# wild-firefox/FreeRL

Hardware: AMD Instinct MI355X
Metric: learner_updates_per_sec (higher is better)
Workload: dtype f32; 1 GPU; TD3.learn() (BASELINE configs[1] algorithm; north_star synthetic shape): obs_dim 8, act_dim 2, batch 256, replay 1e6 rows filled, hidden 128, policy_freq 2, device-drawn indices/noise; learners_per_gpu=512, kernel_family=chained (one eight-wave workgroup per learner, two waves per SIMD), rows_per_workgroup=256, lds_bytes=160128, parallelism=seeds sharded over 1 GPU(s), no data-path collective, collective=metric all-reduce: none (single process)

## Files before the change

### freerl_amd/csrc/frl_api.hip

```cpp
#include <hip/hip_runtime.h>

#include <chrono>
#include <cmath>
#include <cstdarg>
#include <cstdio>
#include <cstdlib>
#include <cstring>
#include <string>
#include <vector>

#include "../../include/freerl_hip.h"
#include "frl_desc.h"

#include "kernels.h"
#ifdef FRL_UNITY
#include "kernels_replay.hip"
#include "kernels_update.hip"
#include "kernels_dqn.hip"
#include "kernels_critic.hip"
#include "kernels_actor.hip"
#include "kernels_act.hip"
#include "kernels_ppo.hip"
#include "kernels_ppo2.hip"
#include "kernels_critic2.hip"
// ... 21 lines not shown
    va_start(ap, fmt);
    vsnprintf(buf, sizeof buf, fmt, ap);
    va_end(ap);
    g_err = buf;
    return code;
}

#define HIP_TRY(expr)                                                                              \
    do {                                                                                           \
        hipError_t _e = (expr);                                                                    \
        if (_e != hipSuccess) return fail(FRL_ERR_HIP, "%s: %s (%s:%d)", #expr, hipGetErrorString(_e), __FILE__, __LINE__); \
    } while (0)

static inline int pad16(int x) { return (x + 15) / 16 * 16; }
static inline int pad32(int x) { return (x + 31) / 32 * 32; }

struct frl_engine {
    frl_config cfg;
    EngineDesc h;
    EngineDesc* d = nullptr;
    hipStream_t stream = nullptr;
    hipEvent_t ev0 = nullptr, ev1 = nullptr, ev_stage = nullptr;
    int lds_bytes = 0;
    std::vector<int> index, size;
    float* stage_rows = nullptr;
    long long* stage_slots = nullptr;
    float* d_stage_rows = nullptr;
    long long* d_stage_slots = nullptr;
    int stage_cap = 0, stage_n = 0;
    bool stage_inflight = false;
    std::vector<int> staged_per_learner;
    int* h_idx = nullptr;
    long long* h_idx64 = nullptr;
    long long* d_idx64 = nullptr;
    float* h_noise = nullptr;
    size_t idx_count = 0, noise_count = 0;
    unsigned long long rng_counter = 0;
    float* d_act_wk = nullptr;
    size_t act_wk_slot = 0;
    std::vector<unsigned long long> act_wk_version;
    unsigned long long param_version = 1;
    float* d_solo_slab = nullptr;
    float* d_solo_part = nullptr;
    unsigned* d_solo_bar = nullptr;
    int* d_solo_err = nullptr;
    int* d_solo_pre = nullptr;
    unsigned solo_pre_seq = 0;
    bool ma_pre_valid = false;
    unsigned long long ma_pre_counter = 0;
    int ma_pre_size = 0, ma_pre_batch = 0;
    int* h_solo_err = nullptr;
    int* d_solo_ticket = nullptr;
    unsigned solo_bar_base = 0;
    int solo_stride = 0;
    int solow_wgs = 0;
    unsigned* d_solow_bar2 = nullptr;
    int solow_row_wgs = 0;
    float* d_act_in = nullptr;
    float* d_act_eps = nullptr;
    float* d_act_out = nullptr;
    float* d_act_logp = nullptr;
    size_t act_in_cap = 0, act_out_cap = 0;
    float* d_ou = nullptr;
    unsigned char* d_ou_flags = nullptr;
    size_t ou_n = 0;
    float* d_ppo = nullptr;
    size_t ppo_cap = 0;
    int* d_perm = nullptr;
    size_t perm_cap = 0;
    bool has_nets = false;
    int noisy_per_set = 0;
    float* h_noisy = nullptr;
    bool per_on = false;
    double* d_per_sum = nullptr;
    double* d_per_max = nullptr;
    float per_alpha = 0.5f, per_eps = 0.01f;
    double per_beta = 0.4, per_beta_inc = 0.001;
    std::vector<int> bucket_cursor;
    std::vector<int> size_flushed;
    int* d_size = nullptr;
    int n_cus = 256;
    int lds_per_cu = 160 * 1024;
    int chain_waves = 8;
    int* stage_bucket = nullptr;
    int* d_stage_bucket = nullptr;
    float* d_per_prio = nullptr;
    double* d_uniforms = nullptr;
    bool profile = false;
    std::vector<hipEvent_t> prof_ev;
    std::vector<int> prof_kind;
    size_t prof_used = 0;
    double prof_ms[8] = {0, 0, 0, 0, 0, 0, 0, 0};
    long long prof_n[8] = {0, 0, 0, 0, 0, 0, 0, 0};
};

enum ProfKind { PK_DRAW = 0, PK_GRAD_CRITIC = 1, PK_ADAM_CRITIC = 2, PK_GRAD_ACTOR = 3, PK_ADAM_ACTOR = 4, PK_SOFT = 5, PK_PPO = 6 };

static void prof_begin(frl_engine* e, int kind) {
    if (!e->profile) return;
    if (e->prof_used + 2 > e->prof_ev.size()) {
        for (int i = 0; i < 2; ++i) { hipEvent_t ev; hipEventCreate(&ev); e->prof_ev.push_back(ev); }
    }
    hipEventRecord(e->prof_ev[e->prof_used], e->stream);
    e->prof_kind.push_back(kind);
}
static void prof_end(frl_engine* e) {
    if (!e->profile) return;
    hipEventRecord(e->prof_ev[e->prof_used + 1], e->stream);
    e->prof_used += 2;
}
static void prof_collect(frl_engine* e) {
    if (e->prof_used == 0) return;
    hipStreamSynchronize(e->stream);
    for (size_t i = 0; i < e->prof_used; i += 2) {
        float ms = 0.f;
        if (hipEventElapsedTime(&ms, e->prof_ev[i], e->prof_ev[i + 1]) == hipSuccess) {
            const int k = e->prof_kind[i / 2];
            e->prof_ms[k] += ms;
            e->prof_n[k]++;
        }
    }
    e->prof_used = 0;
    e->prof_kind.clear();
}

static int build_net(NetDesc& N, const std::vector<std::pair<int, int>>& layers_in , int heads,
                     int hidden_act, int out_act, int extra_n, int n_shadow = 0) {
    memset(&N, 0, sizeof N);
    std::vector<std::pair<int, int>> layers = layers_in;
    for (int i = 0; i < n_shadow; ++i) layers.push_back(layers_in.back());
    N.n_layers = (int)layers.size();
    N.heads = heads;
    N.hidden_act = hidden_act;
    N.out_act = out_act;
    int off = 0, np = 0;
    for (int i = 0; i < N.n_layers; ++i) {
        LayerDesc& L = N.L[i];
        L.n = layers[i].first;
        L.k = layers[i].second;
        L.n_pad = pad16(L.n);
        L.k_pad = pad16(L.k);
        L.w_off = off;
        off += L.n_pad * L.k_pad;
        L.b_off = off;
        off += L.n_pad;
        np += L.n * L.k + L.n;
    }
    N.extra_off = -1;
    N.extra_n = extra_n;
    if (extra_n > 0) {
        N.extra_off = off;
        off += pad16(extra_n);
        np += extra_n;
    }
    N.size = pad32(off);
    N.n_params = np;
    N.n_layers -= n_shadow;
    N.n_shadow = n_shadow;
    return 0;
}

static void build_record(RecordDesc& R, const frl_config& c) {
    memset(&R, 0, sizeof R);
    R.n_agents = c.n_agents;
    int off = 0;
    for (int j = 0; j < c.n_agents; ++j) { R.obs_off[j] = off; R.obs_dim[j] = c.obs_dim[j]; off += c.obs_dim[j]; }
// ... 1073 lines not shown
}

extern "C" int frl_noisy_resample(frl_engine* e, const float* eps_host) {
    ENG(e);
    if (!e->h.noisy) return fail(FRL_ERR_STATE, "engine has no NoisyLinear head");
    if (eps_host) { int rc = noisy_upload(e, eps_host, 0, 1); if (rc) return rc; }
    else hipLaunchKernelGGL(noisy_draw_kernel, dim3(e->h.P, 1), dim3(256), 0, e->stream, e->d, 0, 1, e->rng_counter++);
    hipLaunchKernelGGL(noisy_materialise_kernel, dim3(e->h.P), dim3(256), 0, e->stream, e->d, 0, 1, 0);
    HIP_TRY(hipGetLastError());
    return FRL_OK;
}

static void launch_adam(frl_engine* e, hipStream_t st, const AdamArgs& ad, int units, dim3 grid_adam) {
    const EngineDesc& h = e->h;
    int max_n4 = 0;
    for (int ag = 0; ag < h.n_agents; ++ag) {
        const int net = (h.algo == ALGO_DQN) ? 0 : (ad.which == 0 ? 2 * ag + 1 : 2 * ag);
        max_n4 = std::max(max_n4, h.net[net].size / 4);
    }
    const bool two_pass = getenv("FRL_ADAM_TWO_PASS") != nullptr;
    if (max_n4 <= kFusedThreads * kFusedVec && !h.noisy && !two_pass) {
        hipLaunchKernelGGL(adam_fused_kernel, dim3(units), dim3(kFusedThreads), 0, st, e->d, ad);
    } else if (max_n4 <= kFusedThreads * kFusedVecWide && !two_pass) {
        hipLaunchKernelGGL(adam_fused_wide_kernel, dim3(units), dim3(kFusedThreads), 0, st, e->d, ad);
    } else {
        hipLaunchKernelGGL(reduce_kernel, grid_adam, dim3(256), 0, st, e->d, ad);
        hipLaunchKernelGGL(adam_kernel, grid_adam, dim3(256), 0, st, e->d, ad);
    }
}

static bool chained_shape(const EngineDesc& h) {
    const NetDesc &NA0 = h.net[0], &NC0 = h.net[1];
    auto packed = [](const NetDesc& N) {
        for (int hd = 0; hd < N.heads; ++hd) {
            const LayerDesc* L = N.L + 3 * hd;
            const int b = hd * kHeadFloats;
            if (L[0].w_off != b + kL1w || L[0].b_off != b + kL1b || L[1].w_off != b + kL2w || L[1].b_off != b + kL2b ||
                L[2].w_off != b + kL3w || L[2].b_off != b + kL3b) return false;
        }
        return N.extra_n == 0 || (N.heads == 1 && N.extra_off == kHeadFloats);
    };
    if (NA0.n_layers != 3 || NC0.n_layers != 3 * NC0.heads || h.hidden != 128 || !packed(NA0) || !packed(NC0)) return false;
    if (h.rec.obs_off[0] % 4 != 0 || h.rec.act_off[0] != h.rec.obs_off[0] + h.rec.obs_dim[0] || h.rec.obs_off[0] + 16 > h.rec.stride) return false;
    return (h.algo == ALGO_DDPG || h.algo == ALGO_TD3 || h.algo == ALGO_SAC) && h.n_agents == 1 && h.hidden == 128 &&
           NA0.L[0].k_pad == 16 && NC0.L[0].k_pad == 16 && h.rec.act_dim[0] <= 4 && NA0.L[2].n_pad == 16 &&
           h.batch_max <= 256 && NA0.hidden_act == ACT_RELU && NC0.hidden_act == ACT_RELU &&
           NA0.n_layers == 3 && NC0.n_layers == 3 * NC0.heads;
}
static bool chained_path(const EngineDesc& h, int batch, int pc) {
    (void)pc;
    if (h.wide) return !h.obs_norm_on;
    if (h.solow) return !h.obs_norm_on;
    return h.net[0].frag && h.net[1].frag && batch <= 256 && !h.obs_norm_on;
}
static bool wide_shape(const EngineDesc& h) {
    const bool single = (h.algo == ALGO_DDPG || h.algo == ALGO_TD3 || h.algo == ALGO_SAC) && h.n_agents == 1;
    const bool multi = h.algo == ALGO_MADDPG && h.n_agents >= 1;
    const int H = h.hidden;
    if (!(single || multi) || (H != 128 && H != 256) || h.rec.act_total > kWideApitch) return false;
    if (h.batch_max > 2 * kWideSlice) return false;
    const int nt3 = h.net[0].L[2].n_pad;
    for (int j = 0; j < h.n_agents; ++j) {
        const NetDesc &NA0 = h.net[2 * j], &NC0 = h.net[2 * j + 1];
        if (NA0.n_layers != 3 || NA0.heads != 1 || NC0.n_layers != 3 * NC0.heads || NC0.heads != h.net[1].heads) return false;
        if (NA0.hidden_act != ACT_RELU || NC0.hidden_act != ACT_RELU) return false;
        if (NA0.L[0].k_pad > 16 * kWideMaxKB1 || NC0.L[0].k_pad > 16 * kWideMaxKB1) return false;
        if (NA0.L[2].n_pad != nt3 || nt3 > 32) return false;
        for (int hd = 0; hd < NC0.heads; ++hd)
            if (NC0.L[3 * hd].n_pad != H || NC0.L[3 * hd + 1].n_pad != H || NC0.L[3 * hd + 1].k_pad != H || NC0.L[3 * hd + 2].n_pad != 16) return false;
        if (NA0.L[0].n_pad != H || NA0.L[1].n_pad != H || NA0.L[1].k_pad != H) return false;
    }
    return true;
}

static bool dqn_fused_path(const EngineDesc& h, int batch, bool per_weights) {
    const NetDesc& N = h.net[0];
    (void)per_weights;
    const bool shape = h.algo == ALGO_DQN && !h.noisy && !h.c51_atoms && h.hidden == 128 && N.n_layers == 2 &&
                       N.L[0].k_pad == 16 && N.L[1].n_pad == 16 && batch <= kDqn2Batch && !h.obs_norm_on && N.hidden_act == ACT_RELU;
    const char* force = getenv("FRL_DQN_FUSED");
    return shape && (force ? atoi(force) != 0 : true);
}

static void launch_learn_stage(frl_engine* e, hipStream_t st, LearnArgs a, int stage, int p0, int pc, bool dev_rng, bool needs_noise,
                               const DqnStepArgs* step = nullptr, const SoloStepArgs* sstep = nullptr) {
    const EngineDesc& h = e->h;
    a.p0 = p0; a.p_count = pc;
    const int ns = ((a.batch + h.rc - 1) / h.rc + h.cps - 1) / h.cps;
    const int units = pc * h.n_agents;
    const dim3 grid_chunks(((units + 7) / 8) * 8 * ns), grid_units(units), blk(256), grid_adam(units * h.Gmax);
    const bool sac = h.algo == ALGO_SAC || h.algo == ALGO_SAC_DISCRETE, maddpg = h.algo == ALGO_MADDPG;
    AdamArgs ad;
    memset(&ad, 0, sizeof ad);
    ad.ns = ns; ad.batch = a.batch; ad.eps = a.adam_eps; ad.beta1 = a.beta1; ad.beta2 = a.beta2; ad.clip = a.clip_norm;
    ad.tau = a.tau; ad.alpha_lr = a.alpha_lr; ad.target_entropy = a.target_entropy; ad.p0 = p0; ad.G = h.Gmax;
    const bool v2 = chained_path(h, a.batch, pc);
    if (stage == 0 && dqn_fused_path(h, a.batch, a.use_isw != 0)) {
        a.dqn_split = dqn_split_for(h, a.batch, pc);
        prof_begin(e, PK_GRAD_CRITIC);
        DqnStepArgs sa;
        memset(&sa, 0, sizeof sa);
        if (step) sa = *step;
        hipLaunchKernelGGL(dqn_fused_kernel, dim3(pc * a.dqn_split), blk, (size_t)dqn2_lds_floats() * sizeof(float), st, e->d, a, sa);
        prof_end(e);
        return;
    }
    const int ma_pre_stride = 8 + h.batch_max;
    const bool ma_solow = v2 && h.solow && h.n_agents > 1 && stage == 0 && dev_rng && !needs_noise && pc == h.P;
    const bool ma_use_pre = ma_solow && e->ma_pre_valid && e->ma_pre_counter == a.rng_counter && e->ma_pre_size == a.size && e->ma_pre_batch == a.batch;
    if (stage == 0) {
        if (dev_rng && !ma_use_pre && !(v2 && (h.solo || (h.solow && h.n_agents == 1)))) {
            prof_begin(e, PK_DRAW);
            const char* scan = getenv("FRL_DRAW_SCAN");
            const bool table = a.batch > 256 && 4 * a.batch <= kDrawTableHost && !(scan && atoi(scan) != 0);
            const size_t draw_lds = ((size_t)2 * ((a.batch + 3) & ~3) + (table ? 2 * kDrawTableHost : 0)) * sizeof(int);
            hipLaunchKernelGGL(draw_kernel, grid_units, blk, draw_lds, st, e->d, a, (needs_noise ? 1 : 0) | (table ? 0 : 2));
            prof_end(e);
        }
        if (h.obs_norm_on && h.algo != ALGO_DQN)
            hipLaunchKernelGGL(obsnorm_kernel, dim3(pc), blk, 0, st, e->d, a.batch, 0, p0);
        if (h.noisy)
            hipLaunchKernelGGL(noisy_materialise_kernel, dim3(h.P), blk, 0, st, e->d, 0, 3, 0x2);
        if (v2 && h.wide) {
            prof_begin(e, PK_GRAD_CRITIC);
            const bool x = h.wide == 2;
            const size_t lb = (size_t)(x ? wide16_lds_floats_host() : wide_lds_floats()) * sizeof(float);
            const bool twin = h.net[1].heads == 2, a2 = h.net[0].L[2].n_pad > 16;
            auto k = x ? (twin ? (a2 ? ac_critic_x_h2a2_kernel : ac_critic_x_h2a1_kernel) : (a2 ? ac_critic_x_h1a2_kernel : ac_critic_x_h1a1_kernel))
                       : (twin ? (a2 ? ac_critic_wide_h2a2_kernel : ac_critic_wide_h2a1_kernel) : (a2 ? ac_critic_wide_h1a2_kernel : ac_critic_wide_h1a1_kernel));
            hipLaunchKernelGGL(k, dim3(units), blk, lb, st, e->d, a);
            prof_end(e);
            return;
        }
        if (v2 && h.solow) {
            prof_begin(e, PK_GRAD_CRITIC);
            SoloArgs sa{e->d_solo_slab, e->d_solo_part, e->d_solo_bar, e->d_solo_err, e->solo_bar_base, e->solo_stride, nullptr, nullptr, 0ull, h.solow, e->d_solow_bar2, e->solow_row_wgs, e->solow_wgs};
            e->solo_bar_base += kSoloWG;
            if (dev_rng && e->d_solo_pre && pc == h.P && h.n_agents == 1) {
                const char* pdf = getenv("FRL_SOLO_PREDRAW");
                sa.pre_read = e->d_solo_pre + (size_t)(e->solo_pre_seq & 1) * h.P * kSoloPre;
                if (e->solow_wgs > e->solow_row_wgs && !(pdf && atoi(pdf) == 0)) {
                    sa.pre_write = e->d_solo_pre + (size_t)((e->solo_pre_seq + 1) & 1) * h.P * kSoloPre;
                    sa.pre_counter = e->rng_counter;
                }
                ++e->solo_pre_seq;
            }
            const bool twin = h.net[1].heads == 2, a2 = h.net[0].L[2].n_pad > 16;
            auto k = h.n_agents > 1 ? (twin ? (a2 ? solow_critic_ma_h2a2_kernel : solow_critic_ma_h2a1_kernel) : (a2 ? solow_critic_ma_h1a2_kernel : solow_critic_ma_h1a1_kernel))
                                    : (twin ? (a2 ? solow_critic_h2a2_kernel : solow_critic_h2a1_kernel) : (a2 ? solow_critic_h1a2_kernel : solow_critic_h1a1_kernel));
            if (a.fuse_actor) k = twin ? (a2 ? solow_step_h2a2_kernel : solow_step_h2a1_kernel) : (a2 ? solow_step_h1a2_kernel : solow_step_h1a1_kernel);
            int extra = 0;
            if (h.n_agents > 1) {
                const char* pdf = getenv("FRL_SOLO_PREDRAW");
                if (ma_use_pre) sa.pre_read = e->d_solo_pre + (size_t)(e->solo_pre_seq & 1) * h.P * h.n_agents * ma_pre_stride;
                e->ma_pre_valid = false;
                if (ma_solow && units * (e->solow_wgs + 1) <= e->n_cus && !(pdf && atoi(pdf) == 0)) {
                    sa.pre_write = e->d_solo_pre + (size_t)((e->solo_pre_seq + 1) & 1) * h.P * h.n_agents * ma_pre_stride;
                    sa.pre_counter = e->rng_counter;
                    extra = units;
                    e->ma_pre_valid = true; e->ma_pre_counter = e->rng_counter; e->ma_pre_size = a.size; e->ma_pre_batch = a.batch;
                }
                ++e->solo_pre_seq;
            }
            hipLaunchKernelGGL(k, dim3(units * e->solow_wgs + extra), blk, (size_t)solow_lds_floats() * sizeof(float), st, e->d, a, sa);
            prof_end(e);
            return;
        }
        if (v2 && h.solo) {
            prof_begin(e, PK_GRAD_CRITIC);
            SoloArgs sa{e->d_solo_slab, e->d_solo_part, e->d_solo_bar, e->d_solo_err, e->solo_bar_base, e->solo_stride, nullptr, nullptr, 0ull};
            e->solo_bar_base += kSoloWG;
            SoloStepArgs ss;
            memset(&ss, 0, sizeof ss);
            if (sstep) ss = *sstep;
            const size_t lb = (size_t)std::max(solo_lds_floats(), critic2_lds_floats()) * sizeof(float);
            const char* pdf = getenv("FRL_SOLO_PREDRAW");
            const int W = h.solo;
            const bool predraw = dev_rng && !sstep && e->d_solo_pre && pc == h.P && pc * (W + 1) <= e->n_cus && !(pdf && atoi(pdf) == 0);
            int extra = 0;
            if (dev_rng && !sstep && e->d_solo_pre && pc == h.P) {
                sa.pre_read = e->d_solo_pre + (size_t)(e->solo_pre_seq & 1) * h.P * kSoloPre;
                if (predraw) {
                    sa.pre_write = e->d_solo_pre + (size_t)((e->solo_pre_seq + 1) & 1) * h.P * kSoloPre;
                    sa.pre_counter = e->rng_counter;
                    extra = pc;
                }
                ++e->solo_pre_seq;
            }
            const bool twin = h.net[1].heads == 2;
            auto k = W == 16 ? (twin ? solo_critic_twin_kernel : solo_critic_single_kernel) : (twin ? solo_critic_twin_w8_kernel : solo_critic_single_w8_kernel);
            hipLaunchKernelGGL(k, dim3(pc * W + extra), blk, lb, st, e->d, a, sa, ss);
            prof_end(e);
            return;
        }
        if (v2) {
            { const char* sg = getenv("FRL_STAGGER"); a.stagger = sg ? atoi(sg) : 0;
              const char* gg = getenv("FRL_STAGGER_GROUPS"); a.stagger_groups = gg ? atoi(gg) : 4; a.stagger_wgs = e->n_cus; }
            prof_begin(e, PK_GRAD_CRITIC);
            const bool w8 = e->chain_waves == 8, twin = h.net[1].heads == 2;
            const size_t lb = (size_t)(w8 ? critic8_lds_floats() : critic2_lds_floats()) * sizeof(float);
            const RecordDesc& R = h.rec;
            const bool nv = R.nobs_off[0] % 4 == 0 && R.nobs_off[0] + 16 <= R.stride && R.rew_off % 2 == 0 && R.done_off == R.rew_off + 1 && !getenv("FRL_CRITIC2_NOVEC");
            auto k = w8 ? (nv ? (twin ? ac_critic_v2_twin_nv_kernel : ac_critic_v2_single_nv_kernel) : (twin ? ac_critic_v2_twin_kernel : ac_critic_v2_single_kernel))
                        : (twin ? ac_critic_v2w4_twin_kernel : ac_critic_v2w4_single_kernel);
            hipLaunchKernelGGL(k, dim3(pc), dim3(w8 ? 512 : 256), lb, st, e->d, a);
            prof_end(e);
            return;
        }
        prof_begin(e, PK_GRAD_CRITIC);
        if (h.algo == ALGO_DQN && h.c51_atoms) hipLaunchKernelGGL(c51_grad_kernel, grid_chunks, blk, e->lds_bytes, st, e->d, a, ns);
        else if (h.algo == ALGO_DQN) hipLaunchKernelGGL(dqn_grad_kernel, grid_chunks, blk, e->lds_bytes, st, e->d, a, ns);
        else if (h.algo == ALGO_SAC_DISCRETE) hipLaunchKernelGGL(sacd_critic_kernel, grid_chunks, blk, e->lds_bytes, st, e->d, a, ns);
        else hipLaunchKernelGGL(ac_critic_kernel, grid_chunks, blk, e->lds_bytes, st, e->d, a, ns);
        prof_end(e);
        ad.which = 0; ad.lr = a.critic_lr; ad.wd = a.critic_wd;
        ad.soft = (h.algo == ALGO_DQN) ? 1 : ((!maddpg && a.do_actor) ? 1 : 0);
        prof_begin(e, PK_ADAM_CRITIC);
        launch_adam(e, st, ad, units, grid_adam);
        prof_end(e);
    } else if (stage == 1) {
        if (v2 && h.wide) {
            prof_begin(e, PK_GRAD_ACTOR);
            const bool x = h.wide == 2, a2 = h.net[0].L[2].n_pad > 16;
            auto k = x ? (a2 ? ac_actor_x_a2_kernel : ac_actor_x_a1_kernel) : (a2 ? ac_actor_wide_a2_kernel : ac_actor_wide_a1_kernel);
            hipLaunchKernelGGL(k, dim3(units), blk, (size_t)(x ? wide16_lds_floats_host() : wide_lds_floats()) * sizeof(float), st, e->d, a);
            prof_end(e);
            return;
        }
        if (v2 && h.solow) {
            prof_begin(e, PK_GRAD_ACTOR);
            SoloArgs sa{e->d_solo_slab, e->d_solo_part, e->d_solo_bar, e->d_solo_err, e->solo_bar_base, e->solo_stride, nullptr, nullptr, 0ull, h.solow, e->d_solow_bar2, e->solow_row_wgs, e->solow_wgs};
            e->solo_bar_base += kSoloWG;
            const bool a2 = h.net[0].L[2].n_pad > 16;
            hipLaunchKernelGGL(h.n_agents > 1 ? (a2 ? solow_actor_ma_a2_kernel : solow_actor_ma_a1_kernel) : (a2 ? solow_actor_a2_kernel : solow_actor_a1_kernel), dim3(units * e->solow_wgs), blk,
                               (size_t)solow_lds_floats() * sizeof(float), st, e->d, a, sa);
            prof_end(e);
            return;
        }
        if (v2 && h.solo) {
            prof_begin(e, PK_GRAD_ACTOR);
            SoloArgs sa{e->d_solo_slab, e->d_solo_part, e->d_solo_bar, e->d_solo_err, e->solo_bar_base, e->solo_stride, nullptr, nullptr, 0ull};
            e->solo_bar_base += kSoloWG;
            SoloStepArgs ss;
            memset(&ss, 0, sizeof ss);
            if (sstep) ss = *sstep;
            const int W = h.solo;
            hipLaunchKernelGGL(W == 16 ? solo_actor_kernel : solo_actor_w8_kernel, dim3(pc * W), blk,
                               (size_t)std::max(solo_lds_floats(), critic2_lds_floats()) * sizeof(float), st, e->d, a, sa, ss);
            prof_end(e);
            return;
        }
        if (v2) {
            prof_begin(e, PK_GRAD_ACTOR);
            const bool w8 = e->chain_waves == 8;
            hipLaunchKernelGGL(w8 ? ac_actor_v2_kernel : ac_actor_v2w4_kernel, dim3(pc), dim3(w8 ? 512 : 256),
                               (size_t)(w8 ? critic8_lds_floats() : critic2_lds_floats()) * sizeof(float), st, e->d, a);
            prof_end(e);
            return;
        }
        prof_begin(e, PK_GRAD_ACTOR);
        if (h.algo == ALGO_SAC_DISCRETE) hipLaunchKernelGGL(sacd_actor_kernel, grid_chunks, blk, e->lds_bytes, st, e->d, a, ns);
        else hipLaunchKernelGGL(ac_actor_kernel, grid_chunks, blk, e->lds_bytes, st, e->d, a, ns);
        prof_end(e);
        ad.which = 1; ad.lr = a.actor_lr; ad.wd = 0.f; ad.soft = maddpg ? 0 : 1; ad.sac_alpha = sac ? 1 : 0;
        prof_begin(e, PK_ADAM_ACTOR);
        launch_adam(e, st, ad, units, grid_adam);
        prof_end(e);
    } else {
        prof_begin(e, PK_SOFT);
        int biggest = 0;
        for (int i = 0; i < h.n_nets; ++i) biggest = std::max(biggest, h.net[i].size);
        const int per = std::max(1, std::min((biggest + 4095) / 4096, 4 * e->n_cus / std::max(1, pc * h.n_nets)));
        hipLaunchKernelGGL(soft_update_kernel, dim3(pc * h.n_nets, per), blk, 0, st, e->d, a.tau, p0);
        prof_end(e);
    }
}

static int learn_impl(frl_engine* e, const frl_learn_args* args, const DqnStepArgs* step, const SoloStepArgs* sstep = nullptr, int size_override = -1,
                      hipStream_t stream_override = nullptr) {
    ENG(e);
    if (!args) return fail(FRL_ERR_INVALID, "args is NULL");
    const EngineDesc& h = e->h;
    if (!(h.algo == ALGO_DQN || h.algo == ALGO_DDPG || h.algo == ALGO_TD3 || h.algo == ALGO_SAC || h.algo == ALGO_MADDPG ||
          h.algo == ALGO_SAC_DISCRETE))
        return fail(FRL_ERR_STATE, "frl_learn: engine algo %d has no off-policy learn (PPO: frl_ppo_learn)", h.algo);
    if (args->batch < 1 || args->batch > h.batch_max) return fail(FRL_ERR_INVALID, "batch %d outside [1,%d]", args->batch, h.batch_max);
    int min_size = h.capacity;
    for (int p = 0; p < h.P; ++p) min_size = std::min(min_size, e->size[p]);
    if (size_override >= 0) min_size = size_override;
    if (min_size < args->batch) return fail(FRL_ERR_STATE, "a ring holds %d rows < batch %d", min_size, args->batch);
    if (args->per && (h.algo != ALGO_DQN || !e->per_on)) return fail(FRL_ERR_STATE, "per = 1 needs a DQN engine with frl_per_enable");
    if (args->per && args->idx) return fail(FRL_ERR_INVALID, "per = 1 uses the rows of the last frl_per_sample; idx must be NULL");
    const bool dev_rng = (args->idx == nullptr) && !args->per;
    if (dev_rng && min_size < 2 * args->batch)
        return fail(FRL_ERR_STATE, "device index draw needs len(buffer) >= 2*batch (have %d); pass idx", min_size);
    const bool td3_like = (h.algo == ALGO_TD3 || h.algo == ALGO_MADDPG);
    const bool needs_noise = (h.algo == ALGO_SAC) || (td3_like && args->use_policy_noise);
    if (!dev_rng && needs_noise && !args->noise) return fail(FRL_ERR_INVALID, "idx given without noise: both or neither");
    int rc = flush_stage(e);
    if (rc) return rc;
    rc = upload_idx_noise(e, args->idx, needs_noise ? args->noise : nullptr, args->batch, h.n_agents);
    if (rc) return rc;
    LearnArgs a;
    memset(&a, 0, sizeof a);
    a.batch = args->batch;
    a.size = min_size;
    a.device_rng = dev_rng ? 1 : 0;
    a.do_actor = td3_like ? (args->do_actor ? 1 : 0) : 1;
    a.gamma = args->gamma; a.tau = args->tau;
    a.actor_lr = args->actor_lr; a.critic_lr = args->critic_lr; a.alpha_lr = args->alpha_lr;
    a.adam_eps = args->adam_eps > 0 ? args->adam_eps : 1e-8f;
    a.beta1 = 0.9f; a.beta2 = 0.999f;
    a.critic_wd = args->critic_weight_decay;
    a.clip_norm = args->clip_norm;
    a.policy_noise = args->policy_noise; a.noise_clip = args->noise_clip;
    a.max_action = args->max_action != 0.f ? args->max_action : 1.f;
    a.policy_noise_scale = args->policy_noise_scale;
    a.use_policy_noise = (td3_like && args->use_policy_noise) ? 1 : 0;
    a.target_entropy = args->target_entropy;
    a.double_dqn = (h.algo == ALGO_DQN && args->double_dqn) ? 1 : 0;
    a.use_isw = (h.algo == ALGO_DQN && args->per) ? (args->per == 2 ? 2 : 1) : 0;
    if (args->loss_kind != FRL_LOSS_MSE && args->loss_kind != FRL_LOSS_HUBER) return fail(FRL_ERR_INVALID, "unknown loss_kind %d", args->loss_kind);
    if (args->loss_kind == FRL_LOSS_HUBER) {
        if (!(args->huber_delta > 0.f)) return fail(FRL_ERR_INVALID, "Huber loss needs huber_delta > 0");
        if (h.c51_atoms) return fail(FRL_ERR_STATE, "the Categorical head's loss is a cross-entropy: no Huber variant");
        if (h.algo == ALGO_SAC_DISCRETE) return fail(FRL_ERR_INVALID, "discrete SAC's critic loss is F.mse_loss (SAC_add_discrete.py:313-314): no Huber variant");
        a.huber = 1; a.huber_delta = args->huber_delta;
    }
    a.rng_counter = e->rng_counter++;
    ++e->param_version;
    const bool actor_stage = (h.algo != ALGO_DQN && a.do_actor), soft_stage = (h.algo == ALGO_MADDPG && a.do_actor && !(h.solow && chained_path(h, a.batch, h.P)));
    if (h.noisy) {
        const int first = a.double_dqn ? 0 : 1;
        if (args->noisy_eps) { rc = noisy_upload(e, args->noisy_eps, first, 3 - first); if (rc) return rc; }
        else hipLaunchKernelGGL(noisy_draw_kernel, dim3(h.P, 3), dim3(256), 0, e->stream, e->d, 0, 3, e->rng_counter++);
// ... 323 lines not shown
```

### freerl_amd/csrc/frl_desc.h

```cpp
#pragma once
#include <stdint.h>

namespace frl {

constexpr int kMaxLayers = 6;
constexpr int kMaxAgents = 8;
constexpr int kMaxNets = 2 * kMaxAgents;

enum Act : int { ACT_NONE = 0, ACT_RELU = 1, ACT_TANH = 2 };
enum Algo : int { ALGO_DQN = 0, ALGO_DDPG = 1, ALGO_TD3 = 2, ALGO_SAC = 3, ALGO_MADDPG = 4, ALGO_PPO = 5, ALGO_SAC_DISCRETE = 6 };

struct LayerDesc {
    int n, k;
    int n_pad, k_pad;
    int w_off, b_off;
};

struct NetDesc {
    int n_layers;
    int size;
    int n_params;
    int hidden_act;
    int out_act;
    int extra_off;
// ... 55 lines not shown
};

struct EngineDesc {
    int algo, P, n_agents, hidden, rc;
    int capacity;
    int batch_max;
    int n_nets;
    int learner_stride;
    int net_off[kMaxNets];
    NetDesc net[kMaxNets];
    RecordDesc rec;
    float* theta;
    float* target;
    float* m;
    float* v;
    float* grad;
    float* slab;
    float* act_spill;
    float* part;
    int S;
    int cps;
    float* gsq;
    int Gmax;
    float* replay;
    int* idx;
    float* noise;
    int noise_sets;
    float* stats;
    int* steps;
    int* ticket;
    float* alpha;
    unsigned long long seed;
    int act_max;
    int lds_kin_pad, lds_out_pad, lds_batch_pad, lds_act_pad;
    int lds_hbufs;
    int n_discrete;
    float* isw;
    float* td_err;
    int noisy;
    int noisy_split;
    float* theta_eff;
    float* noisy_eps;
    int c51_atoms;
    float c51_vmin, c51_vmax;
    int dueling;
    int cat_logits;
    int beta_actor;
    float* obsnorm;
    int obs_norm_on;
    int obsnorm_w;
    int wide;
    int wide_bm;
    int wide_xp, wide_op;
    int wide_unit;
    float* wide_scr;
    int solow;
    int solo;
};

struct LearnArgs {
    int batch;
    int size;
    int device_rng;
    int do_actor;
    float gamma, tau;
    float actor_lr, critic_lr, alpha_lr;
    float adam_eps, beta1, beta2;
    float critic_wd;
    float clip_norm;
    float policy_noise, noise_clip, max_action, policy_noise_scale;
    int use_policy_noise;
    float target_entropy;
    unsigned long long rng_counter;
    int p0, p_count;
    int double_dqn;
    int use_isw;
    int dqn_split;
    int stagger;
    int stagger_groups;
    int stagger_wgs;
    int fuse_actor;
    int huber;
    float huber_delta;
};

}
```

### freerl_amd/csrc/kernels_actor2.hip

```cpp
#include <hip/hip_runtime.h>

#include "kernels.h"
#include "device/chain_net.hpp"
#include "device/update_common.hpp"
#include "device/ppo_timing.hpp"

namespace frl {

template <int NW, int TA>
__device__ __forceinline__ void ac_actor_v2_body(const EngineDesc& D, const LearnArgs& a, float* smem) {
    constexpr int kRC = 16 * NW, kRowsT = kRC * TA;
    constexpr int kNC = kChainBatch / kRC, kNCT = kChainBatch / kRowsT;
    static_assert(kNCT >= 1, "a chunk of passes A / B is at most the whole batch");
    const int p = a.p0 + blockIdx.x;
    const RecordDesc& R = D.rec;
    const NetDesc& NA = D.net[0];
    const NetDesc& NC = D.net[1];
    using Net = ChainNetT<NW>;
    Net C;
    C.init(smem);
    const ChainLds& S = C.S;
    const int tid = C.tid, l = C.l, w = C.w, i16 = C.i16, q = C.q;
    const int B = a.batch, O = R.obs_dim[0], A = R.act_dim[0];
    const size_t lbase = (size_t)p * D.learner_stride;
    g_f thA = as_global(D.theta + lbase + D.net_off[0]);
    g_f tgA = as_global(D.target + lbase + D.net_off[0]);
    g_f mA = as_global(D.m + lbase + D.net_off[0]);
    g_f vA = as_global(D.v + lbase + D.net_off[0]);
    g_cf thC = as_global(D.theta + lbase + D.net_off[1]);
    g_cf ring = as_global(D.replay + (size_t)p * D.capacity * R.stride);
    g_ci idx = as_global_i(D.idx + (size_t)p * D.batch_max);
    const float invB = 1.f / (float)B;
    const bool sac = (D.algo == ALGO_SAC);
    const float alpha = sac ? D.alpha[p * 4 + 3] : 0.f;
    const int am = D.act_max;
    g_cf noise1 = as_global(D.noise + ((size_t)p * D.noise_sets + 1) * D.batch_max * am);
    const int nq = sac ? NC.heads : 1;
    const float dqv = sac ? -0.5f * invB : -invB;
    const int nchunks = (B + kRC - 1) / kRC, nch2 = (B + kRowsT - 1) / kRowsT;
    lds_f dab = S.eb;

    int ridxT[kNC], ridx[kNC];
#pragma unroll
    for (int j4 = 0; j4 < kNC; ++j4) {
        const int rowT = (j4 / TA) * kRowsT + 16 * TA * w + (j4 % TA) * 16 + i16, row = j4 * kRC + 16 * w + i16;
        ridxT[j4] = rowT < B ? idx[rowT] : -1;
        ridx[j4] = row < B ? idx[row] : -1;
    }
    struct RowIn2 { f32x4 x[TA]; };
    auto load_obs2 = [&](int c2) {
        RowIn2 X;
#pragma unroll
        for (int t = 0; t < TA; ++t) {
            X.x[t] = f32x4{0.f, 0.f, 0.f, 0.f};
            int ri = ridxT[t];
#pragma unroll
            for (int cc = 1; cc < kNCT; ++cc) ri = c2 == cc ? ridxT[TA * cc + t] : ri;
            if (ri >= 0) {
                g_cf rec = ring + (size_t)ri * R.stride;
#pragma unroll
                for (int e = 0; e < 4; ++e)
                    if (4 * q + e < O) X.x[t][e] = rec[R.obs_off[0] + 4 * q + e];
            }
        }
        return X;
    };
    auto load_obs = [&](int c) {
        f32x4 x = {0.f, 0.f, 0.f, 0.f};
        const int ri = pick(ridx, c);
        if (ri >= 0) {
            g_cf rec = ring + (size_t)ri * R.stride;
#pragma unroll
            for (int e = 0; e < 4; ++e)
                if (4 * q + e < O) x[e] = rec[R.obs_off[0] + 4 * q + e];
        }
        return x;
    };

    float lpsum = 0.f;
    PPO_T0();
    RowIn2 nxt2 = load_obs2(0);
    typename Net::StageRegs pend = C.stage_fetch((g_cf)thA, 0, NA.extra_n);
    C.stage_commit(pend);
    PPO_T(0);
    for (int c2 = 0; c2 < nch2; ++c2) {
        const RowIn2 cur = nxt2;
        nxt2 = load_obs2(c2 + 1 < nch2 ? c2 + 1 : 0);
        if (c2 + 1 == nch2) pend = C.stage_fetch(thC, 0);
        f32x4 z[TA], h1[TA][kHT], h2[TA][kHT];
        C.template forward_vh<TA>(cur.x, h1, h2, z, A);
#pragma unroll
        for (int t = 0; t < TA; ++t) {
            const int row = c2 * kRowsT + 16 * TA * w + 16 * t + i16;
            if (q == 0 && row < kChainBatch) {
                f32x4 an = {0.f, 0.f, 0.f, 0.f};
#pragma unroll
                for (int r = 0; r < 4; ++r) {
                    if (r < A && row < B) {
                        if (sac) {
                            const float ls = fminf(fmaxf(S.ls[r], -20.f), 2.f), sd = expf(ls);
                            const float u = z[t][r] + sd * noise1[(size_t)row * am + r], du = u - z[t][r];
                            lpsum += -(du * du) / (2.f * sd * sd) - ls - kLogSqrt2Pi;
                            lpsum -= 2.f * (kLog2 - u - softplus_t(-2.f * u));
                            an[r] = tanhf(u);
                        } else {
                            an[r] = tanhf(z[t][r]);
                        }
                    }
                }
                st4(S.ab + row * 4, an);
            }
        }
    }
    float qsum = 0.f;
    f32x4 nxt;
    PPO_T(1);
    for (int hd = 0; hd < nq; ++hd) {
        C.stage_commit(pend);
        PPO_T(0);
        for (int c2 = 0; c2 < nch2; ++c2) {
            const RowIn2 cur = nxt2;
            if (c2 + 1 < nch2) nxt2 = load_obs2(c2 + 1);
            else if (hd + 1 < nq) nxt2 = load_obs2(0);
            else nxt = load_obs(0);
            f32x4 xb[TA], z[TA], h1[TA][kHT], h2[TA][kHT];
#pragma unroll
            for (int t = 0; t < TA; ++t) {
                const int row = c2 * kRowsT + 16 * TA * w + 16 * t + i16;
                xb[t] = cur.x[t];
#pragma unroll
                for (int e = 0; e < 4; ++e) {
                    const int f = 4 * q + e;
                    if (row < B && f >= O && f < O + A) xb[t][e] = S.ab[row * 4 + f - O];
                }
            }
            C.template forward_vh<TA>(xb, h1, h2, z, 1);
#pragma unroll
            for (int t = 0; t < TA; ++t) {
                const int row = c2 * kRowsT + 16 * TA * w + 16 * t + i16;
                const bool valid = row < B;
                f32x4 dz = {0.f, 0.f, 0.f, 0.f};
                if (q == 0 && valid) { qsum += z[t][0]; dz[0] = dqv; }
                f32x4 d2[kHT], d1[kHT];
                C.delta2_valu(dz, h2[t], d2, 1);
                C.delta1(d2, h1[t], d1);
                const f32x4 dx = C.delta0(d1);
#pragma unroll
                for (int r = 0; r < 4; ++r) {
                    const int f = 4 * q + r;
                    if (valid && f >= O && f < O + A) dab[row * 4 + f - O] = hd == 0 ? dx[r] : dab[row * 4 + f - O] + dx[r];
                }
            }
        }
        pend = hd + 1 < nq ? C.stage_fetch(thC, hd + 1) : C.stage_fetch((g_cf)thA, 0, NA.extra_n);
        PPO_T(2);
    }
    typename Net::Grad g;
    PPO_T(2);
    C.grad_zero(g);
    C.stage_commit(pend);
    PPO_T(0);
    f32x4 dqa[kNC], epsa[kNC], ava[NW == 8 ? kNC : 1];
#pragma unroll
    for (int c = 0; c < kNC; ++c) {
        const int row = c * kRC + 16 * w + i16;
        dqa[c] = (q == 0 && row < B) ? ld4((lds_cf)(dab + row * 4)) : f32x4{0.f, 0.f, 0.f, 0.f};
        if constexpr (NW == 8) ava[c] = (q == 0 && row < B) ? ld4((lds_cf)(S.ab + row * 4)) : f32x4{0.f, 0.f, 0.f, 0.f};
        epsa[c] = f32x4{0.f, 0.f, 0.f, 0.f};
        if (sac && q == 0 && row < B) {
#pragma unroll
            for (int r = 0; r < 4; ++r)
                if (r < A) epsa[c][r] = noise1[(size_t)row * am + r];
        }
    }
    float gls[4] = {0.f, 0.f, 0.f, 0.f};
    for (int c = 0; c < nchunks; ++c) {
        const int row = c * kRC + 16 * w + i16;
        f32x4 xb[1] = {nxt}, z[1], h1[1][kHT], h2[1][kHT];
        nxt = load_obs(c + 1 < nchunks ? c + 1 : 0);
        PPO_T(5);
        C.template forward_vh<1>(xb, h1, h2, z, A);
        PPO_T(3);
        const f32x4 dq = pick(dqa, c);
        f32x4 dz = {0.f, 0.f, 0.f, 0.f};
        if (q == 0 && row < B) {
            if (sac) {
                const f32x4 ep = pick(epsa, c);
                f32x4 av4;
                if constexpr (NW == 8) av4 = pick(ava, c); else av4 = ld4((lds_cf)(S.ab + row * 4));
#pragma unroll
                for (int r = 0; r < 4; ++r) {
                    if (r < A) {
                        const float av = av4[r];
                        const float d = dq[r] * (1.f - av * av) + (alpha * invB) * (2.f * av);
                        const float ls = fminf(fmaxf(S.ls[r], -20.f), 2.f);
                        dz[r] = d;
                        gls[r] += d * expf(ls) * ep[r] - alpha * invB;
                    }
                }
            } else {
#pragma unroll
                for (int r = 0; r < 4; ++r)
                    if (r < A) { const float av = tanhf(z[0][r]); dz[r] = dq[r] * (1.f - av * av); }
            }
        }
        C.backward(g, xb[0], h1[0], h2[0], dz, A);
        PPO_T(4);
    }
    C.grad_finish(g);
    float ss = wave_sum(C.grad_sumsq(g));
    const float qs = wave_sum(qsum), lps = wave_sum(lpsum);
#pragma unroll
    for (int r = 0; r < 4; ++r) gls[r] = wave_sum(gls[r]);
    lds_barrier();
    if (l == 0) {
        S.red[w] = ss; S.red[8 + w] = qs; S.red[16 + w] = lps;
#pragma unroll
        for (int r = 0; r < 4; ++r) S.red[24 + 8 * r + w] = gls[r];
    }
    int* steps = D.steps + (size_t)p * (kMaxNets + 1);
    if (tid == 0) S.red[56] = __int_as_float(steps[0]);
    lds_barrier();
    auto red_sum = [&](int base) {
        float v = S.red[base];
#pragma unroll
        for (int i = 1; i < NW; ++i) v += S.red[base + i];
        return v;
    };
    float g_extra = 0.f, ss_extra = 0.f;
    if (sac) {
#pragma unroll
        for (int r = 0; r < 4; ++r) {
            if (r < A) {
                const float raw = S.ls[r];
                const float gr = (raw >= -20.f && raw <= 2.f) ? red_sum(24 + 8 * r) : 0.f;
                ss_extra += gr * gr;
                if (i16 == r) g_extra = gr;
            }
        }
    }
    const float total = sqrtf(red_sum(0) + ss_extra);
    const float qtot = red_sum(8);
    const float lptot = red_sum(16);
    const int t = __float_as_int(S.red[56]) + 1;
    const double bc1 = 1.0 - powi_d((double)a.beta1, t), bc2 = 1.0 - powi_d((double)a.beta2, t);
    AdamCoef co;
    co.coef = a.clip_norm > 0.f ? fminf(a.clip_norm / (total + 1e-6f), 1.f) : 1.f;
    co.step = (float)((double)a.actor_lr / bc1); co.inv_bc2s = 1.f / (float)sqrt(bc2);
    co.w1 = 1.f - a.beta1; co.w2 = 1.f - a.beta2; co.beta2 = a.beta2; co.eps = a.adam_eps; co.wd = 0.f;
    co.tk = 1.f - a.tau; co.tau = a.tau;
    PPO_T(5);
    C.template adam_head<true, 0, true>(g, thA, mA, vA, tgA, co, g_extra, sac ? NA.extra_n : 0);
    PPO_T(6);
    PPO_TDUMP();
    if (tid == 0) {
        steps[0] = t;
        float* st = D.stats + (size_t)p * ST_COUNT;
        st[ST_ACTOR_LOSS] = actor_loss_stat(sac, qtot, lptot, alpha, invB);
        st[ST_ACTOR_GNORM] = total;
        if (sac) sac_alpha_step(D.alpha + p * 4, st, steps, alpha, -lptot * invB, a.target_entropy, a.beta1, a.beta2, a.alpha_lr);
    }
// ... 16 lines not shown
```

### freerl_amd/csrc/kernels_critic2.hip

```cpp
#include <hip/hip_runtime.h>

#include "kernels.h"
#include "device/chain_net.hpp"
#include "device/update_common.hpp"
#include "device/ppo_timing.hpp"

#if defined(FRL_BWD_TIMING)
#undef PPO_UDUMP
#define PPO_UDUMP() do {} while (0)
#endif

namespace frl {

#ifndef FRL_CRITIC2_TT
#define FRL_CRITIC2_TT 2
#endif
#ifndef FRL_CRITIC2_AHEAD
#define FRL_CRITIC2_AHEAD 1
#endif
template <bool TWIN, int TT, int NW, bool NVEC>
__device__ __forceinline__ void ac_critic_v2_body(const EngineDesc& D, const LearnArgs& a, float* smem) {
    constexpr int kRC = 16 * NW;
    constexpr int kRowsT = kRC * TT;
    constexpr int kNC = kChainBatch / kRC;
    constexpr int kNCT = kChainBatch / kRowsT;
    static_assert(kNCT >= 1, "a target-pass chunk is at most the whole batch");
    constexpr int NH = TWIN ? 2 : 1;
    const int p = a.p0 + blockIdx.x;
    const RecordDesc& R = D.rec;
    const NetDesc& NA = D.net[0];
    const NetDesc& NC = D.net[1];
    using Net = ChainNetT<NW>;
    Net C;
    C.init(smem);
    const ChainLds& S = C.S;
    const int tid = C.tid, l = C.l, w = C.w, i16 = C.i16, q = C.q;
    const int B = a.batch, O = R.obs_dim[0], A = R.act_dim[0], am = D.act_max;
    const bool sac = (D.algo == ALGO_SAC);
    const size_t lbase = (size_t)p * D.learner_stride;
    g_cf tgA = as_global(D.target + lbase + D.net_off[0]);
    g_cf tgC = as_global(D.target + lbase + D.net_off[1]);
    g_f thC = as_global(D.theta + lbase + D.net_off[1]);
    g_f tgCw = as_global(D.target + lbase + D.net_off[1]);
    g_f mC = as_global(D.m + lbase + D.net_off[1]);
    g_f vC = as_global(D.v + lbase + D.net_off[1]);
    g_cf ring = as_global(D.replay + (size_t)p * D.capacity * R.stride);
    g_ci idx = as_global_i(D.idx + (size_t)p * D.batch_max);
    g_cf noise0 = as_global(D.noise + (size_t)p * D.noise_sets * D.batch_max * am);
    const float alpha = sac ? D.alpha[p * 4 + 3] : 0.f;
    const float invB = 1.f / (float)B;
    const int nchunks = (B + kRC - 1) / kRC;

    int ridx[kNC];
#pragma unroll
    for (int c = 0; c < kNC; ++c) {
        const int row = c * kRC + 16 * w + i16;
        ridx[c] = idx[row < B ? row : B - 1];
    }
    const int xoff = R.obs_off[0] + 4 * q;
    struct RowIn { f32x4 x; };
    auto load_row = [&](int c) {
        RowIn X;
        X.x = ld4(ring + (size_t)pick(ridx, c) * R.stride + xoff);
        return X;
    };
    auto zero_pad = [&](const f32x4& x, int width) {
        f32x4 r;
#pragma unroll
        for (int e = 0; e < 4; ++e) r[e] = 4 * q + e < width ? x[e] : 0.f;
        return r;
    };
    int ridxT[kNC];
#pragma unroll
    for (int j4 = 0; j4 < kNC; ++j4) {
        const int row = (j4 / TT) * kRowsT + 16 * TT * w + (j4 % TT) * 16 + i16;
        ridxT[j4] = idx[row < B ? row : B - 1];
    }
    int colo[4];
#pragma unroll
    for (int e = 0; e < 4; ++e) colo[e] = R.nobs_off[0] + (NVEC ? 4 * q : (4 * q + e < O ? 4 * q + e : O - 1));
    struct RowIn2 { f32x4 x[TT]; float rew[TT], done[TT]; };
    auto tile_of = [&](const int (&v)[kNC], int c2, int t) {
        int r = v[t];
#pragma unroll
        for (int cc = 1; cc < kNCT; ++cc) r = c2 == cc ? v[TT * cc + t] : r;
        return r;
    };
    auto load_row2 = [&](bool want_rd, int c2) {
        RowIn2 X;
#pragma unroll
        for (int t = 0; t < TT; ++t) {
            g_cf rec = ring + (size_t)tile_of(ridxT, c2, t) * R.stride;
            if constexpr (NVEC) {
                typedef float f32x2 __attribute__((ext_vector_type(2)));
                X.x[t] = ld4(rec + colo[0]);
                const f32x2 rd = *reinterpret_cast<const FRL_GLB f32x2*>(rec + R.rew_off);
                X.rew[t] = rd[0]; X.done[t] = rd[1];
            } else {
#pragma unroll
                for (int e = 0; e < 4; ++e) X.x[t][e] = rec[colo[e]];
                X.rew[t] = rec[R.rew_off]; X.done[t] = rec[R.done_off];
            }
        }
        return X;
    };
    const int nch2 = (B + kRowsT - 1) / kRowsT;

    if (a.stagger > 0 && (int)blockIdx.x < a.stagger_wgs) {
        const int group = (blockIdx.x >> 3) & (a.stagger_groups - 1);
        for (int i = 0; i < group * a.stagger; ++i) __builtin_amdgcn_s_sleep(32);
    }
// ... 218 lines not shown
```

Before: 818,300 updates/s.

## Alternate learner order across chained launches and prefetch actor inputs earlier

Critic and actor chained kernels now map blocks to learners in alternating forward/reverse order between consecutive launches, presumably so learners that finish last in one launch start first in the next, or to reuse cache contents. The actor kernel also prefetches SAC noise into registers up front, replaces guarded scalar observation loads with unconditional vector loads that are masked afterwards, and issues the next weight-stage fetch during the last chunk's backward pass to overlap it with compute. The added costs are register pressure from the noise array and out-of-range clamped index reads.

```diff
diff --git a/freerl_amd/csrc/frl_api.hip b/freerl_amd/csrc/frl_api.hip
--- a/freerl_amd/csrc/frl_api.hip
+++ b/freerl_amd/csrc/frl_api.hip
@@ -127,6 +127,8 @@
     int n_cus = 256;
     int lds_per_cu = 160 * 1024;
     int chain_waves = 8;
+    bool chain_reverse = false;
+    int chain_last_stage = -1;
     int* stage_bucket = nullptr;
     int* d_stage_bucket = nullptr;
     float* d_per_prio = nullptr;
@@ -1366,6 +1368,16 @@
     return shape && (force ? atoi(force) != 0 : true);
 }
 
+#ifndef FRL_CHAIN_ORDER
+#define FRL_CHAIN_ORDER 1
+#endif
+static int chain_direction(frl_engine* e, int stage) {
+    if (FRL_CHAIN_ORDER == 1) { if (e->chain_last_stage >= 0) e->chain_reverse = !e->chain_reverse; }
+    else if (FRL_CHAIN_ORDER == 2) { if (stage == 0 && e->chain_last_stage == 0) e->chain_reverse = !e->chain_reverse; }
+    e->chain_last_stage = stage;
+    return e->chain_reverse ? 1 : 0;
+}
+
 static void launch_learn_stage(frl_engine* e, hipStream_t st, LearnArgs a, int stage, int p0, int pc, bool dev_rng, bool needs_noise,
                                const DqnStepArgs* step = nullptr, const SoloStepArgs* sstep = nullptr) {
     const EngineDesc& h = e->h;
@@ -1480,6 +1492,7 @@
         if (v2) {
             { const char* sg = getenv("FRL_STAGGER"); a.stagger = sg ? atoi(sg) : 0;
               const char* gg = getenv("FRL_STAGGER_GROUPS"); a.stagger_groups = gg ? atoi(gg) : 4; a.stagger_wgs = e->n_cus; }
+            a.reverse = chain_direction(e, 0);
             prof_begin(e, PK_GRAD_CRITIC);
             const bool w8 = e->chain_waves == 8, twin = h.net[1].heads == 2;
             const size_t lb = (size_t)(w8 ? critic8_lds_floats() : critic2_lds_floats()) * sizeof(float);
@@ -1535,6 +1548,7 @@
             return;
         }
         if (v2) {
+            a.reverse = chain_direction(e, 1);
             prof_begin(e, PK_GRAD_ACTOR);
             const bool w8 = e->chain_waves == 8;
             hipLaunchKernelGGL(w8 ? ac_actor_v2_kernel : ac_actor_v2w4_kernel, dim3(pc), dim3(w8 ? 512 : 256),
diff --git a/freerl_amd/csrc/frl_desc.h b/freerl_amd/csrc/frl_desc.h
--- a/freerl_amd/csrc/frl_desc.h
+++ b/freerl_amd/csrc/frl_desc.h
@@ -161,6 +161,7 @@
     int fuse_actor;
     int huber;
     float huber_delta;
+    int reverse;
 };
 
 }
diff --git a/freerl_amd/csrc/kernels_actor2.hip b/freerl_amd/csrc/kernels_actor2.hip
--- a/freerl_amd/csrc/kernels_actor2.hip
+++ b/freerl_amd/csrc/kernels_actor2.hip
@@ -4,6 +4,13 @@
 #include "device/chain_net.hpp"
 #include "device/update_common.hpp"
 #include "device/ppo_timing.hpp"
+
+#ifndef FRL_ACTOR2_NZ_AHEAD
+#define FRL_ACTOR2_NZ_AHEAD 1
+#endif
+#ifndef FRL_ACTOR2_FETCH_UNDER_B
+#define FRL_ACTOR2_FETCH_UNDER_B 1
+#endif
 
 namespace frl {
 
@@ -12,7 +19,7 @@
     constexpr int kRC = 16 * NW, kRowsT = kRC * TA;
     constexpr int kNC = kChainBatch / kRC, kNCT = kChainBatch / kRowsT;
     static_assert(kNCT >= 1, "a chunk of passes A / B is at most the whole batch");
-    const int p = a.p0 + blockIdx.x;
+    const int p = a.p0 + (a.reverse ? (int)gridDim.x - 1 - (int)blockIdx.x : (int)blockIdx.x);
     const RecordDesc& R = D.rec;
     const NetDesc& NA = D.net[0];
     const NetDesc& NC = D.net[1];
@@ -44,62 +51,79 @@
 #pragma unroll
     for (int j4 = 0; j4 < kNC; ++j4) {
         const int rowT = (j4 / TA) * kRowsT + 16 * TA * w + (j4 % TA) * 16 + i16, row = j4 * kRC + 16 * w + i16;
-        ridxT[j4] = rowT < B ? idx[rowT] : -1;
-        ridx[j4] = row < B ? idx[row] : -1;
-    }
+        ridxT[j4] = idx[rowT < B ? rowT : B - 1];
+        ridx[j4] = idx[row < B ? row : B - 1];
+    }
+    const int xoff = R.obs_off[0] + 4 * q;
     struct RowIn2 { f32x4 x[TA]; };
     auto load_obs2 = [&](int c2) {
         RowIn2 X;
 #pragma unroll
         for (int t = 0; t < TA; ++t) {
-            X.x[t] = f32x4{0.f, 0.f, 0.f, 0.f};
             int ri = ridxT[t];
 #pragma unroll
             for (int cc = 1; cc < kNCT; ++cc) ri = c2 == cc ? ridxT[TA * cc + t] : ri;
-            if (ri >= 0) {
-                g_cf rec = ring + (size_t)ri * R.stride;
-#pragma unroll
-                for (int e = 0; e < 4; ++e)
-                    if (4 * q + e < O) X.x[t][e] = rec[R.obs_off[0] + 4 * q + e];
-            }
+            X.x[t] = ld4(ring + (size_t)ri * R.stride + xoff);
         }
         return X;
     };
-    auto load_obs = [&](int c) {
-        f32x4 x = {0.f, 0.f, 0.f, 0.f};
-        const int ri = pick(ridx, c);
-        if (ri >= 0) {
-            g_cf rec = ring + (size_t)ri * R.stride;
-#pragma unroll
-            for (int e = 0; e < 4; ++e)
-                if (4 * q + e < O) x[e] = rec[R.obs_off[0] + 4 * q + e];
-        }
-        return x;
+    auto load_obs = [&](int c) { return ld4(ring + (size_t)pick(ridx, c) * R.stride + xoff); };
+    auto obs_in = [&](const f32x4& x, int row) {
+        f32x4 r;
+#pragma unroll
+        for (int e = 0; e < 4; ++e) r[e] = (row < B && 4 * q + e < O) ? x[e] : 0.f;
+        return r;
     };
 
     float lpsum = 0.f;
     PPO_T0();
     RowIn2 nxt2 = load_obs2(0);
+#if FRL_ACTOR2_NZ_AHEAD
+    f32x4 nzr[kNC];
+#pragma unroll
+    for (int j4 = 0; j4 < kNC; ++j4) {
+        nzr[j4] = f32x4{0.f, 0.f, 0.f, 0.f};
+        const int row = (j4 / TA) * kRowsT + 16 * TA * w + (j4 % TA) * 16 + i16;
+        if (sac && q == 0 && row < B) {
+#pragma unroll
+            for (int r = 0; r < 4; ++r)
+                if (r < A) nzr[j4][r] = noise1[(size_t)row * am + r];
+        }
+    }
+#endif
     typename Net::StageRegs pend = C.stage_fetch((g_cf)thA, 0, NA.extra_n);
     C.stage_commit(pend);
     PPO_T(0);
-    for (int c2 = 0; c2 < nch2; ++c2) {
+    auto actor_chunk = [&](int c2, auto last_c) {
+        constexpr bool last = decltype(last_c)::value;
         const RowIn2 cur = nxt2;
-        nxt2 = load_obs2(c2 + 1 < nch2 ? c2 + 1 : 0);
-        if (c2 + 1 == nch2) pend = C.stage_fetch(thC, 0);
-        f32x4 z[TA], h1[TA][kHT], h2[TA][kHT];
-        C.template forward_vh<TA>(cur.x, h1, h2, z, A);
+        nxt2 = load_obs2(last ? 0 : c2 + 1);
+        if constexpr (last) pend = C.stage_fetch(thC, 0);
+        f32x4 xo[TA], z[TA], h1[TA][kHT], h2[TA][kHT];
+#pragma unroll
+        for (int t = 0; t < TA; ++t) xo[t] = obs_in(cur.x[t], c2 * kRowsT + 16 * TA * w + 16 * t + i16);
+        C.template forward_vh<TA>(xo, h1, h2, z, A);
 #pragma unroll
         for (int t = 0; t < TA; ++t) {
             const int row = c2 * kRowsT + 16 * TA * w + 16 * t + i16;
             if (q == 0 && row < kChainBatch) {
                 f32x4 an = {0.f, 0.f, 0.f, 0.f};
+#if FRL_ACTOR2_NZ_AHEAD
+                f32x4 nr = nzr[t];
+#pragma unroll
+                for (int cc = 1; cc < kNCT; ++cc) nr = c2 == cc ? nzr[TA * cc + t] : nr;
+#endif
 #pragma unroll
                 for (int r = 0; r < 4; ++r) {
                     if (r < A && row < B) {
                         if (sac) {
                             const float ls = fminf(fmaxf(S.ls[r], -20.f), 2.f), sd = expf(ls);
-                            const float u = z[t][r] + sd * noise1[(size_t)row * am + r], du = u - z[t][r];
+#if FRL_ACTOR2_NZ_AHEAD
+                            const float ep = nr[r];
+#else
+                            const float ep = noise1[(size_t)row * am + r];
+#endif
+                            const float u = z[t][r] + sd * ep, du = u - z[t][r];
                             lpsum += -(du * du) / (2.f * sd * sd) - ls - kLogSqrt2Pi;
                             lpsum -= 2.f * (kLog2 - u - softplus_t(-2.f * u));
                             an[r] = tanhf(u);
@@ -111,23 +135,28 @@
                 st4(S.ab + row * 4, an);
             }
         }
-    }
+    };
+    for (int c2 = 0; c2 + 1 < nch2; ++c2) actor_chunk(c2, IC<0>{});
+    actor_chunk(nch2 - 1, IC<1>{});
     float qsum = 0.f;
     f32x4 nxt;
     PPO_T(1);
     for (int hd = 0; hd < nq; ++hd) {
         C.stage_commit(pend);
         PPO_T(0);
-        for (int c2 = 0; c2 < nch2; ++c2) {
+        const bool more = hd + 1 < nq;
+        g_cf nth = more ? thC + (hd + 1) * kHeadFloats : (g_cf)thA;
+        const int nextra = more ? 0 : NA.extra_n;
+        auto q_chunk = [&](int c2, auto last_c) {
+            constexpr bool last = decltype(last_c)::value;
             const RowIn2 cur = nxt2;
-            if (c2 + 1 < nch2) nxt2 = load_obs2(c2 + 1);
-            else if (hd + 1 < nq) nxt2 = load_obs2(0);
-            else nxt = load_obs(0);
+            if constexpr (!last) nxt2 = load_obs2(c2 + 1);
+            else { nxt2 = load_obs2(0); nxt = load_obs(0); }
             f32x4 xb[TA], z[TA], h1[TA][kHT], h2[TA][kHT];
 #pragma unroll
             for (int t = 0; t < TA; ++t) {
                 const int row = c2 * kRowsT + 16 * TA * w + 16 * t + i16;
-                xb[t] = cur.x[t];
+                xb[t] = obs_in(cur.x[t], row);
 #pragma unroll
                 for (int e = 0; e < 4; ++e) {
                     const int f = 4 * q + e;
@@ -144,6 +173,9 @@
                 f32x4 d2[kHT], d1[kHT];
                 C.delta2_valu(dz, h2[t], d2, 1);
                 C.delta1(d2, h1[t], d1);
+#if FRL_ACTOR2_FETCH_UNDER_B
+                if constexpr (last && NW == 8) { if (t == TA - 1) pend = C.stage_fetch(nth, 0, nextra); }
+#endif
                 const f32x4 dx = C.delta0(d1);
 #pragma unroll
                 for (int r = 0; r < 4; ++r) {
@@ -151,8 +183,10 @@
                     if (valid && f >= O && f < O + A) dab[row * 4 + f - O] = hd == 0 ? dx[r] : dab[row * 4 + f - O] + dx[r];
                 }
             }
-        }
-        pend = hd + 1 < nq ? C.stage_fetch(thC, hd + 1) : C.stage_fetch((g_cf)thA, 0, NA.extra_n);
+        };
+        for (int c2 = 0; c2 + 1 < nch2; ++c2) q_chunk(c2, IC<0>{});
+        q_chunk(nch2 - 1, IC<1>{});
+        if constexpr (!(FRL_ACTOR2_FETCH_UNDER_B && NW == 8)) pend = C.stage_fetch(nth, 0, nextra);
         PPO_T(2);
     }
     typename Net::Grad g;
@@ -176,7 +210,7 @@
     float gls[4] = {0.f, 0.f, 0.f, 0.f};
     for (int c = 0; c < nchunks; ++c) {
         const int row = c * kRC + 16 * w + i16;
-        f32x4 xb[1] = {nxt}, z[1], h1[1][kHT], h2[1][kHT];
+        f32x4 xb[1] = {obs_in(nxt, row)}, z[1], h1[1][kHT], h2[1][kHT];
         nxt = load_obs(c + 1 < nchunks ? c + 1 : 0);
         PPO_T(5);
         C.template forward_vh<1>(xb, h1, h2, z, A);
diff --git a/freerl_amd/csrc/kernels_critic2.hip b/freerl_amd/csrc/kernels_critic2.hip
--- a/freerl_amd/csrc/kernels_critic2.hip
+++ b/freerl_amd/csrc/kernels_critic2.hip
@@ -26,7 +26,7 @@
     constexpr int kNCT = kChainBatch / kRowsT;
     static_assert(kNCT >= 1, "a target-pass chunk is at most the whole batch");
     constexpr int NH = TWIN ? 2 : 1;
-    const int p = a.p0 + blockIdx.x;
+    const int p = a.p0 + (a.reverse ? (int)gridDim.x - 1 - (int)blockIdx.x : (int)blockIdx.x);
     const RecordDesc& R = D.rec;
     const NetDesc& NA = D.net[0];
     const NetDesc& NC = D.net[1];
```

Result: no change. 820,800 updates/s (median of 6 runs) (+0.3%).
